# Whisper-6/DynamicTreeAttn

Hardware: AMD Instinct MI355X
Metric: tree-attn fwd+bwd tokens/sec, Qwen3-0.6B tau2-16k tries (higher is better)
Workload: dtype bf16

## Files before the change

### dynamictreeattn_amd/_lib.py

```python
from __future__ import annotations

import ctypes as C
import os

from .build import LIB

_lib = None
_i32, _i64, _f32, _vp = C.c_int32, C.c_int64, C.c_float, C.c_void_p

_PROTOS = {
    "dta_version": ([], C.c_int),
    "dta_take_pending_error": ([C.c_char_p, _i32], C.c_int),
    "dta_lcp_adjacent": ([_vp, _vp, _vp, _i32, _vp, _vp, _vp], C.c_int),
    "dta_leafize": ([_vp, _vp, _i32, _vp, _vp, _vp, _vp, _vp], C.c_int),
    "dta_preorder_meta": ([_vp] * 8 + [_i32, _i32] + [_vp] * 4 + [_vp], C.c_int),
    "dta_tree_attn_fwd": ([_vp] * 8 + [_i32] * 6 + [_i64] * 8 + [_f32, _i32] + [_vp, _i32, _f32, _vp], C.c_int),
    "dta_tree_attn_bwd": ([_vp] * 14 + [_i32] * 6 + [_i64] * 12 + [_f32, _i32, _i32, _i32] + [_vp, _i32, _vp, _i32, _vp]
                          + [_vp, _i32, _f32, _vp], C.c_int),
    "dta_window_lo": ([_vp] * 4 + [_i32, _i32, _i32, _vp, _vp], C.c_int),
    "dta_logprob_entropy_fwd": ([_vp] * 8 + [_i32, _i32, _i64, _f32, _i32, _f32, _vp], C.c_int),
    "dta_logprob_entropy_shard_stats": ([_vp] * 6 + [_i32, _i32, _i64, _f32, _i32, _f32, _vp], C.c_int),
    "dta_logprob_entropy_bwd": ([_vp] * 10 + [_i32, _i32, _i64, _i64, _f32, _i32, _f32, _vp], C.c_int),
    "dta_rmsnorm_fwd": ([_vp] * 6 + [_i32, _i32, _f32, _f32, _i32, _vp], C.c_int),
    "dta_rmsnorm_bwd_blocks": ([_i32], C.c_int),
    "dta_rmsnorm_bwd": ([_vp] * 7 + [_i32, _i32, _f32, _i32, _vp], C.c_int),
    "dta_qk_norm_rope_fwd": ([_vp] * 5 + [_i32, _i32, _i32, _i64, _f32, _i32, _vp], C.c_int),
    "dta_qk_norm_rope_bwd_blocks": ([_i64], C.c_int),
    "dta_qk_norm_rope_bwd": ([_vp] * 7 + [_i32, _i32, _i32, _i64, _i64, _i64, _i64, _i32, _vp], C.c_int),
    "dta_wide_qk_norm_rope_fwd": ([_vp] * 5 + [_i32, _i32, _i32, _i64, _f32, _i32, _vp], C.c_int),
    "dta_wide_qk_norm_rope_bwd_blocks": ([_i32], C.c_int),
    "dta_wide_qk_norm_rope_bwd": ([_vp] * 7 + [_i32, _i32, _i32, _i64, _i64, _i64, _i64, _i32, _vp], C.c_int),
    "dta_rmsnorm_add_fwd": ([_vp] * 6 + [_i32, _i32, _f32, _i32, _vp], C.c_int),
    "dta_swiglu_fwd": ([_vp] * 3 + [_i64, _i32, _i64, _i32, _vp], C.c_int),
    "dta_swiglu_bwd": ([_vp] * 5 + [_i64, _i32, _i64, _i64, _i32, _vp], C.c_int),
    "dta_geglu_fwd": ([_vp] * 3 + [_i64, _i32, _i64, _i32, _vp], C.c_int),
    "dta_geglu_bwd": ([_vp] * 5 + [_i64, _i32, _i64, _i64, _i32, _vp], C.c_int),
    "dta_transpose": ([_vp, _vp, _i64, _i64, _i64, _i64, _i32, _vp], C.c_int),
    "dta_sum_slabs": ([_vp, _i64, _i64, _i64, _vp, _vp, _i32, _vp], C.c_int),
    "dta_moe_router_fwd": ([_vp] * 4 + [_i32] * 5 + [_vp], C.c_int),
    "dta_moe_router_bwd": ([_vp] * 5 + [_i32] * 5 + [_vp], C.c_int),
    "dta_moe_permute_workspace": ([_i32, _i32], C.c_int),
    "dta_moe_tile_bound": ([_i32, _i32], C.c_int),
    "dta_moe_permute": ([_vp, _i32, _i32, _i32] + [_vp] * 5 + [_vp], C.c_int),
    "dta_moe_grouped_gemm": ([_i32] + [_vp] * 7 + [_i32] * 5 + [_vp], C.c_int),
    "dta_moe_combine_fwd": ([_vp] * 4 + [_i32] * 4 + [_vp], C.c_int),
    "dta_moe_combine_bwd": ([_vp] * 6 + [_i32] * 4 + [_vp], C.c_int),
    "dta_lora_down": ([_vp, _i64, _vp, _i64, _vp, _i64, _vp, _i32, _i32, _i32, _i32, _vp], C.c_int),
    "dta_lora_wgrad_slabs": ([_i32, _i32], C.c_int),
    "dta_lora_wgrad": ([_vp, _i64, _vp, _i64, _vp, _vp, _i32, _i32, _i32, _i32, _vp], C.c_int),
}
EXPORTS = tuple(_PROTOS)
_ERR = {-1: "DTA_EINVAL", -2: "DTA_EUNSUPPORTED", -3: "DTA_EALIGN", -4: "DTA_ELAUNCH", -5: "DTA_EPRIOR"}


def _hip_runtimes_mapped():
    try:
        with open("/proc/self/maps") as f:
            return sorted({line.split()[-1] for line in f if "libamdhip64" in line})
    except OSError:
        return []

# ... 34 lines not shown
```

### dynamictreeattn_amd/csrc/elementwise_kernels.hip

```cpp
#include <hip/hip_runtime.h>
#include <stdint.h>
#include "dta_common.h"
#include "dta_device.h"

#ifndef DTA_EW_NT
#define DTA_EW_NT 1
#endif
#if DTA_EW_NT
#define DTA_SAVED_LOAD(P) __builtin_nontemporal_load(P)
#else
#define DTA_SAVED_LOAD(P) (*(P))
#endif

namespace {


template <int DT, int NA, bool OFF = false>
__global__ __launch_bounds__(256) void rmsnorm_fwd_kernel(const void* __restrict__ x_, const void* __restrict__ delta_, const void* __restrict__ w_,
                                                          void* __restrict__ xout_, void* __restrict__ y_,
                                                          float* __restrict__ rstd, int R, int H, float eps, float w_off = 0.f) {
  using e = typename Ty<DT>::e; using v8 = typename Ty<DT>::v8;
  const int lane = threadIdx.x & 63, wave = threadIdx.x >> 6;
  const e* w = reinterpret_cast<const e*>(w_);
  const int nv = H >> 3;
// ... 135 lines not shown
    }
  }
  if (!dw_part) return;
  float* out = dw_part + (int64_t)blockIdx.x * H;
#pragma unroll
  for (int a = 0; a < NA; ++a) {
    if (a < per_lane) {
      __syncthreads();
#pragma unroll
      for (int j = 0; j < 8; ++j) red[(wave * 64 + lane) * 8 + j] = acc[a][j];
      __syncthreads();
      if (wave == 0) {
        const int i = lane + 64 * a;
        if (i < nv) {
#pragma unroll
          for (int j = 0; j < 8; ++j) out[8 * i + j] = red[lane * 8 + j] + red[(64 + lane) * 8 + j] + red[(128 + lane) * 8 + j] + red[(192 + lane) * 8 + j];
        }
      }
    }
  }
}

template <int DT, int HPL, int D>
__global__ __launch_bounds__(256) void qk_norm_rope_fwd_kernel(const void* __restrict__ x_, const void* __restrict__ w_, const float* __restrict__ cs,
                                                               void* __restrict__ y_, float* __restrict__ rstd, int64_t n_units, int NH,
                                                               int64_t x_st, float eps) {
  using e = typename Ty<DT>::e; using v8 = typename Ty<DT>::v8;
  constexpr int LPH = D / 8, LSH = D == 128 ? 4 : 3;
  const int lane = threadIdx.x & 63, sub = lane & (LPH - 1);
  const int64_t unit = ((int64_t)blockIdx.x * 4 + (threadIdx.x >> 6)) * (64 / LPH) + (lane >> LSH);
  if (unit >= n_units) return;
  const int groups = NH / HPL;
  const int64_t tok = unit / groups; const int head0 = (int)(unit - tok * groups) * HPL;
  const e* x = reinterpret_cast<const e*>(x_) + tok * x_st + (int64_t)head0 * D + 8 * sub;
  const int64_t hid0 = tok * NH + head0;
  e* y = reinterpret_cast<e*>(y_) + hid0 * D + 8 * sub;
  v8 v[HPL];
#pragma unroll
  for (int h = 0; h < HPL; ++h) v[h] = *reinterpret_cast<const v8*>(x + h * D);
  const float* c = cs + tok * D + 8 * (sub & (LPH / 2 - 1));
  float cj[8], sj[8];
#pragma unroll
  for (int j = 0; j < 8; ++j) { cj[j] = c[j]; sj[j] = sub < LPH / 2 ? -c[D / 2 + j] : c[D / 2 + j]; }
  v8 wv;
  if (w_) wv = *reinterpret_cast<const v8*>(reinterpret_cast<const e*>(w_) + 8 * sub);
#pragma unroll
  for (int h = 0; h < HPL; ++h) {
    float a[8];
    if (w_) {
      float ss = 0.f;
#pragma unroll
      for (int j = 0; j < 8; ++j) { const float f = (float)v[h][j]; ss = __builtin_fmaf(f, f, ss); }
#pragma unroll
      for (int o = LPH / 2; o > 0; o >>= 1) ss += __shfl_xor(ss, o);
      const float r = __builtin_amdgcn_rsqf(ss * (1.f / D) + eps);
      if (sub == 0) rstd[hid0 + h] = r;
#pragma unroll
      for (int j = 0; j < 8; ++j) { const e t = (e)((float)v[h][j] * r); a[j] = (float)(e)((float)wv[j] * (float)t); }
    } else {
#pragma unroll
      for (int j = 0; j < 8; ++j) a[j] = (float)v[h][j];
    }
    v8 o;
#pragma unroll
    for (int j = 0; j < 8; ++j) {
      const float other = __shfl_xor(a[j], LPH / 2);
      o[j] = (e)(a[j] * cj[j] + other * sj[j]);
    }
    *reinterpret_cast<v8*>(y + h * D) = o;
  }
}

template <int DT, int HPL, int D>
__global__ __launch_bounds__(256) void qk_norm_rope_bwd_kernel(const void* __restrict__ x_, const void* __restrict__ w_, const float* __restrict__ cs,
                                                               const void* dy_, const float* __restrict__ rstd,
                                                               void* dx_, float* __restrict__ dw_part, int64_t n_units, int NH,
                                                               int64_t x_st, int64_t dy_st_t, int64_t dy_st_h, int64_t dx_st) {
  using e = typename Ty<DT>::e; using v8 = typename Ty<DT>::v8;
  constexpr int LPH = D / 8, LSH = D == 128 ? 4 : 3, UPB = 4 * (64 / LPH);
  __shared__ float red[256 * 8];
  const int lane = threadIdx.x & 63, sub = lane & (LPH - 1);
  const int groups = NH / HPL;
  float acc[8];
#pragma unroll
  for (int j = 0; j < 8; ++j) acc[j] = 0.f;
  v8 wv;
  if (w_) wv = *reinterpret_cast<const v8*>(reinterpret_cast<const e*>(w_) + 8 * sub);
  for (int64_t base = (int64_t)blockIdx.x * UPB; base < n_units; base += (int64_t)gridDim.x * UPB) {
    const int64_t unit = base + (threadIdx.x >> 6) * (64 / LPH) + (lane >> LSH);
    const bool live = unit < n_units;
    const int64_t uc = live ? unit : n_units - 1;
    const int64_t tok = uc / groups; const int head0 = (int)(uc - tok * groups) * HPL;
    const e* dy = reinterpret_cast<const e*>(dy_) + tok * dy_st_t + (int64_t)head0 * dy_st_h + 8 * sub;
    v8 g[HPL], v[HPL];
#pragma unroll
    for (int h = 0; h < HPL; ++h) g[h] = *reinterpret_cast<const v8*>(dy + h * dy_st_h);
    if (w_) {
      const e* x = reinterpret_cast<const e*>(x_) + tok * x_st + (int64_t)head0 * D + 8 * sub;
#pragma unroll
      for (int h = 0; h < HPL; ++h) v[h] = DTA_SAVED_LOAD(reinterpret_cast<const v8*>(x + h * D));
    }
    const float* c = cs + tok * D + 8 * (sub & (LPH / 2 - 1));
    float cj[8], sj[8];
#pragma unroll
    for (int j = 0; j < 8; ++j) { cj[j] = c[j]; sj[j] = sub < LPH / 2 ? c[D / 2 + j] : -c[D / 2 + j]; }
    e* dx = reinterpret_cast<e*>(dx_) + tok * dx_st + (int64_t)head0 * D + 8 * sub;
#pragma unroll
    for (int h = 0; h < HPL; ++h) {
      float da[8];
#pragma unroll
      for (int j = 0; j < 8; ++j) {
// ... 7 lines not shown
        float dot = 0.f, t[8];
#pragma unroll
        for (int j = 0; j < 8; ++j) { t[j] = (float)v[h][j] * r; dot = __builtin_fmaf(da[j] * (float)wv[j], t[j], dot); if (live) acc[j] = __builtin_fmaf(da[j], t[j], acc[j]); }
#pragma unroll
        for (int o2 = LPH / 2; o2 > 0; o2 >>= 1) dot += __shfl_xor(dot, o2);
        dot *= (1.f / D);
#pragma unroll
        for (int j = 0; j < 8; ++j) o[j] = (e)(r * (da[j] * (float)wv[j] - t[j] * dot));
      } else {
#pragma unroll
        for (int j = 0; j < 8; ++j) o[j] = (e)da[j];
      }
      if (live) *reinterpret_cast<v8*>(dx + h * D) = o;
    }
  }
  if (w_ && dw_part) {
#pragma unroll
    for (int j = 0; j < 8; ++j) red[threadIdx.x * 8 + j] = acc[j];
    __syncthreads();
    if (threadIdx.x < D) {
      const int s = threadIdx.x >> 3, j = threadIdx.x & 7;
      float t = 0.f;
      for (int g2 = 0; g2 < 256 / LPH; ++g2) t += red[(g2 * LPH + s) * 8 + j];
      dw_part[(int64_t)blockIdx.x * D + threadIdx.x] = t;
    }
  }
}

template <int WPT> __device__ __forceinline__ float token_sum(float v, float* slot) {
  v = wave_sum(v);
  if constexpr (WPT == 1) return v;
  else {
    if ((threadIdx.x & 63) == 0) slot[threadIdx.x >> 6] = v;
    __syncthreads();
    const float t = (slot[0] + slot[1]) + (slot[2] + slot[3]);
    __syncthreads();
    return t;
  }
}

template <int DT, int NA, int D, int WPT>
__global__ __launch_bounds__(256) void wide_qk_norm_rope_fwd_kernel(const void* __restrict__ x_, const void* __restrict__ w_, const float* __restrict__ cs,
                                                                    void* __restrict__ y_, float* __restrict__ rstd, int T, int n,
                                                                    int64_t x_st, float eps) {
  using e = typename Ty<DT>::e; using v8 = typename Ty<DT>::v8;
  constexpr int LPH = D / 8, L = 64 * WPT, TPB = 4 / WPT;
  __shared__ float slot[4];
  const int lane = WPT == 1 ? (threadIdx.x & 63) : threadIdx.x, sub = lane & (LPH - 1);
  const e* w = reinterpret_cast<const e*>(w_);
// ... 355 lines not shown
  if (wave == 0 && col < n) {
    float t = extra ? extra[col] : 0.f;
#pragma unroll
    for (int w = 0; w < 16; ++w) t += red[w * 64 + lane];
    reinterpret_cast<e*>(out_)[col] = (e)t;
  }
}
template <int DT>
__global__ __launch_bounds__(256) void sum_slabs_flat_kernel(const float* __restrict__ part, int slabs, int64_t n4, int64_t stride,
                                                             const float* __restrict__ extra, void* __restrict__ out_) {
  using e = typename Ty<DT>::e;
  typedef float f4 __attribute__((ext_vector_type(4)));
  typedef e e4 __attribute__((ext_vector_type(4)));
  for (int64_t i = (int64_t)blockIdx.x * 256 + threadIdx.x; i < n4; i += (int64_t)gridDim.x * 256) {
    f4 t = extra ? *reinterpret_cast<const f4*>(extra + 4 * i) : f4{0.f, 0.f, 0.f, 0.f};
    for (int s2 = 0; s2 < slabs; ++s2) t += *reinterpret_cast<const f4*>(part + s2 * stride + 4 * i);
    e4 o;
#pragma unroll
    for (int j = 0; j < 4; ++j) o[j] = (e)t[j];
    *reinterpret_cast<e4*>(reinterpret_cast<e*>(out_) + 4 * i) = o;
  }
}

template <int N> using Int = std::integral_constant<int, N>;

template <int WIDE, class F> inline void rms_form(int H, float w_offset, F&& f) {
  auto by_h = [&](auto off) {
    if (H <= 1024) f(Int<2>{}, off);
    else if (H <= 2048) f(Int<4>{}, off);
    else if (H <= 4096) f(Int<8>{}, off);
    else f(Int<WIDE>{}, off);
  };
  if (w_offset != 0.f) by_h(std::true_type{}); else by_h(std::false_type{});
}

template <class F> inline void qk_form(int NH, int head_dim, F&& f) {
  if (head_dim == 64) { if (NH % 4 == 0) f(Int<4>{}, Int<64>{}); else f(Int<1>{}, Int<64>{}); }
  else if (NH % 4 == 0) f(Int<4>{}, Int<128>{}); else f(Int<1>{}, Int<128>{});
}

template <class F> inline void wide_qk_form(int64_t n, int head_dim, F&& f) {
  auto by_n = [&](auto d) {
    if (n <= 1024) f(Int<2>{}, d, Int<1>{});
    else if (n <= 2048) f(Int<4>{}, d, Int<1>{});
    else if (n <= 4096) f(Int<2>{}, d, Int<4>{});
    else f(Int<4>{}, d, Int<4>{});
// ... 81 lines not shown
      hipLaunchKernelGGL((qk_norm_rope_fwd_kernel<decltype(dt)::value, HPL, D>), grid, block, 0, st_, x, w, cos_sin, y, rstd, n, NH, x_stride_t, eps);
    });
  });
  return DTA_LAUNCH_STATUS();
}

extern "C" int dta_qk_norm_rope_bwd_blocks(int64_t n_heads_total) { return row_blocks(n_heads_total, 16, 1024); }
extern "C" int dta_qk_norm_rope_bwd(const void* x, const void* w, const float* cos_sin, const void* dy, const float* rstd,
                                    void* dx, float* dw_partial, int32_t T, int32_t NH, int32_t head_dim,
                                    int64_t x_stride_t, int64_t dy_stride_t, int64_t dy_stride_h, int64_t dx_stride_t, int32_t dtype, void* stream) {
  if (!cos_sin || !dy || !dx || T <= 0 || NH <= 0 || (w && (!x || !rstd))) return DTA_EINVAL;
  if (!row_dtype_ok(dtype) || (head_dim != 128 && head_dim != 64)) return DTA_EUNSUPPORTED;
  if (!aligned16(dy) || !aligned16(dx) || (w && (!aligned16(w) || !aligned16(x))) || x_stride_t % 8 || dy_stride_t % 8 || dy_stride_h % 8 || dx_stride_t % 8) return DTA_EALIGN;
  if (dx_stride_t < (int64_t)NH * head_dim) return DTA_EINVAL;
  hipStream_t st_ = static_cast<hipStream_t>(stream);
  DTA_REFUSE_IF_PRIOR_ERROR();
  const dim3 grid(row_blocks((int64_t)T * NH, 16, 1024)), block(256);
  qk_form(NH, head_dim, [&](auto hpl, auto d) {
    constexpr int HPL = decltype(hpl)::value, D = decltype(d)::value;
    const int64_t n = (int64_t)T * (NH / HPL);
    dta_storage_type(dtype, [&](auto dt) {
      hipLaunchKernelGGL((qk_norm_rope_bwd_kernel<decltype(dt)::value, HPL, D>), grid, block, 0, st_, x, w, cos_sin, dy, rstd, dx, dw_partial, n, NH,
                         x_stride_t, dy_stride_t, dy_stride_h, dx_stride_t);
    });
  });
  return DTA_LAUNCH_STATUS();
}

extern "C" int dta_wide_qk_norm_rope_fwd(const void* x, const void* w, const float* cos_sin, void* y, float* rstd,
                                         int32_t T, int32_t NH, int32_t head_dim, int64_t x_stride_t, float eps, int32_t dtype, void* stream) {
  if (!x || !w || !cos_sin || !y || !rstd || T <= 0 || NH <= 0 || eps != eps) return DTA_EINVAL;
  if (!row_dtype_ok(dtype) || (head_dim != 128 && head_dim != 64) || (int64_t)NH * head_dim > 8192) return DTA_EUNSUPPORTED;
  if (!aligned16(x) || !aligned16(w) || !aligned16(y) || x_stride_t % 8) return DTA_EALIGN;
  const int n = NH * head_dim;
  if (x_stride_t < n) return DTA_EINVAL;
  hipStream_t st_ = static_cast<hipStream_t>(stream);
  DTA_REFUSE_IF_PRIOR_ERROR();
  const dim3 grid(row_blocks(T, 4, 8192)), block(256);
  wide_qk_form(n, head_dim, [&](auto na, auto d, auto wpt) {
    dta_storage_type(dtype, [&](auto dt) {
      hipLaunchKernelGGL((wide_qk_norm_rope_fwd_kernel<decltype(dt)::value, decltype(na)::value, decltype(d)::value, decltype(wpt)::value>), grid, block, 0, st_,
                         x, w, cos_sin, y, rstd, T, n, x_stride_t, eps);
    });
  });
  return DTA_LAUNCH_STATUS();
}
// ... 67 lines not shown
}

extern "C" int dta_sum_slabs(const float* part, int64_t slabs, int64_t n, int64_t slab_stride, const float* extra, void* out, int32_t out_dtype,
                             void* stream) {
  if (!part || !out || slabs <= 0 || n <= 0 || slab_stride < n) return DTA_EINVAL;
  if (!row_dtype_ok(out_dtype)) return DTA_EUNSUPPORTED;
  hipStream_t st_ = static_cast<hipStream_t>(stream);
  DTA_REFUSE_IF_PRIOR_ERROR();
  const bool flat = slabs <= 16 && n % 4 == 0 && slab_stride % 4 == 0 && aligned16(part) && aligned16(out) && (!extra || aligned16(extra));
  if (flat) {
    const dim3 grid(row_blocks(n / 4, 256, 8192)), block(256);
    dta_storage_type(out_dtype, [&](auto dt) {
      hipLaunchKernelGGL(sum_slabs_flat_kernel<decltype(dt)::value>, grid, block, 0, st_, part, (int)slabs, n / 4, slab_stride, extra, out);
    });
  } else {
    if ((n + 63) / 64 > 0x7fffffff) return DTA_EUNSUPPORTED;
    const dim3 grid((unsigned)((n + 63) / 64)), block(1024);
    dta_storage_type(out_dtype, [&](auto dt) {
      hipLaunchKernelGGL(sum_slabs_tall_kernel<decltype(dt)::value>, grid, block, 0, st_, part, slabs, n, slab_stride, extra, out);
    });
  }
  return DTA_LAUNCH_STATUS();
}
```

### dynamictreeattn_amd/ops.py

```python
from __future__ import annotations

import math
from dataclasses import dataclass
from typing import Optional

import numpy as np
import torch
import torch.nn.functional as F

from . import packing
from ._lib import check, lib, ptr

_DT = {torch.bfloat16: 0, torch.float16: 1, torch.float32: 2}


class _on:
    __slots__ = ("dev", "_guard")

    def __init__(self, *ts):
        dev = None
        for t in ts:
            if t is None:
                continue
            if not t.is_cuda:
# ... 603 lines not shown
    return sum_slabs(part, w.dtype) if part is not None else None


def _qk_norm_rope_fwd(x, w, cos_sin, eps):
    T, NH, D = x.shape
    y = torch.empty((T, NH, D), dtype=x.dtype, device=x.device)
    rstd = torch.empty(T * NH, dtype=torch.float32, device=x.device) if w is not None else None
    _launch("dta_qk_norm_rope_fwd", (x, w, cos_sin), ptr(x), ptr(w), ptr(cos_sin), ptr(y), ptr(rstd), T, NH, D, x.stride(0), float(eps),
            _DT[x.dtype], nbytes=2 * T * NH * D * x.element_size() + T * D * 4)
    return y, rstd


def _qk_norm_rope_bwd(x, w, cos_sin, dy, rstd, dx, need_w):
    T, NH, D = x.shape
    if dy.stride(2) != 1:
        dy = dy.contiguous()
    part = torch.empty(lib().dta_qk_norm_rope_bwd_blocks(T * NH), D, dtype=torch.float32, device=x.device) if w is not None and need_w else None
    _launch("dta_qk_norm_rope_bwd", (x, cos_sin, dy), ptr(x), ptr(w), ptr(cos_sin), ptr(dy), ptr(rstd) if w is not None else None,
            ptr(dx), ptr(part), T, NH, D, x.stride(0), dy.stride(0), dy.stride(1), dx.stride(0), _DT[x.dtype],
            nbytes=(3 if w is not None else 2) * T * NH * D * x.element_size() + T * D * 4)
    return sum_slabs(part, w.dtype) if part is not None else None


class _QKNormRope(torch.autograd.Function):
    @staticmethod
    def forward(ctx, x, w, cos_sin, eps):
        _require_cuda(x, cos_sin)
        T, NH, D = x.shape
        if x.stride(2) != 1 or x.stride(1) != D:
            x = x.contiguous()
        y, rstd = _qk_norm_rope_fwd(x, w, cos_sin, eps)
        ctx.save_for_backward(x, w if w is not None else cos_sin, cos_sin, rstd if rstd is not None else cos_sin)
        ctx.has_w = w is not None
        return y

    @staticmethod
    def backward(ctx, dy):
        x, w, cos_sin, rstd = ctx.saved_tensors
        dx = torch.empty(x.shape, dtype=x.dtype, device=x.device)
        dw = _qk_norm_rope_bwd(x, w if ctx.has_w else None, cos_sin, dy, rstd, dx, ctx.needs_input_grad[1])
        return dx, dw, None, None


class _QKVPrep(torch.autograd.Function):

    @staticmethod
    def forward(ctx, qkv, wq, wk, cos_sin, eps, Hq, Hkv, wide=False):
        _require_cuda(qkv, cos_sin)
        T, H3, D = qkv.shape
        assert H3 == Hq + 2 * Hkv and qkv.is_contiguous()
        assert not wide or (wq is not None and wk is not None)
        ctx.wide = bool(wide)
        fwd = _wide_qk_norm_rope_fwd if wide else _qk_norm_rope_fwd
        outs, rstds = [], []
        for x, w in ((qkv[:, :Hq], wq), (qkv[:, Hq:Hq + Hkv], wk)):
            y, rstd = fwd(x, w, cos_sin, eps)
            outs.append(y); rstds.append(rstd if rstd is not None else cos_sin)
        ctx.save_for_backward(qkv, wq if wq is not None else cos_sin, wk if wk is not None else cos_sin, cos_sin, rstds[0], rstds[1])
        ctx.has_w = (wq is not None, wk is not None)
        ctx.heads = (Hq, Hkv)
        return outs[0], outs[1], qkv[:, Hq + Hkv:]

    @staticmethod
    def backward(ctx, dq, dk, dv):
        qkv, wq, wk, cos_sin, rq, rk = ctx.saved_tensors
        Hq, Hkv = ctx.heads
        T, H3, D = qkv.shape
        base = dv._base
        in_place = (base is not None and dq._base is base and dk._base is base and base.shape == qkv.shape and base.is_contiguous()
                    and base.dtype == qkv.dtype and dq.shape == (T, Hq, D) and dk.shape == (T, Hkv, D) and dv.shape == (T, Hkv, D)
                    and dq.stride() == dk.stride() == dv.stride() == (H3 * D, D, 1)
                    and (dq.storage_offset(), dk.storage_offset(), dv.storage_offset()) == (0, Hq * D, (Hq + Hkv) * D))
        d = base if in_place else torch.empty_like(qkv)
        dws = []
        for lo, NH, w, rstd, has_w, need_w, dy in ((0, Hq, wq, rq, ctx.has_w[0], ctx.needs_input_grad[1], dq),
                                                   (Hq, Hkv, wk, rk, ctx.has_w[1], ctx.needs_input_grad[2], dk)):
            bwd = _wide_qk_norm_rope_bwd if ctx.wide else _qk_norm_rope_bwd
            dws.append(bwd(qkv[:, lo:lo + NH], w if has_w else None, cos_sin, dy, rstd, d[:, lo:lo + NH], need_w))
        if not in_place:
            d[:, Hq + Hkv:].copy_(dv)
        return d, dws[0], dws[1], None, None, None, None, None


def qkv_prep(qkv: torch.Tensor, wq: Optional[torch.Tensor], wk: Optional[torch.Tensor], cos_sin: torch.Tensor, eps: float,
             Hq: int, Hkv: int):
    return _QKVPrep.apply(qkv, wq, wk, cos_sin, eps, Hq, Hkv)


def qkv_prep_wide(qkv: torch.Tensor, wq: torch.Tensor, wk: torch.Tensor, cos_sin: torch.Tensor, eps: float, Hq: int, Hkv: int):
    return _QKVPrep.apply(qkv, wq, wk, cos_sin, eps, Hq, Hkv, True)


def qk_norm_rope(x: torch.Tensor, w: Optional[torch.Tensor], cos_sin: torch.Tensor, eps: float) -> torch.Tensor:
    return _QKNormRope.apply(x, w, cos_sin, eps)


ROPE_TYPES = ("default", "linear", "llama3", "yarn")


def rope_inv_freq(D: int, rope_parameters: dict, max_position_embeddings: Optional[int] = None):
    rp = rope_parameters
# ... 168 lines not shown
        outs, o = [], 0
        for r in ctx.rows:
            outs.append(g[o:o + r]); o += r
        return tuple(outs)


def stack_rows(*ws: torch.Tensor) -> torch.Tensor:
    return _StackRows.apply(*ws)


def clear_stack_rows_cache() -> None:
    _StackRows._cache.clear(); _StackRows._cached_bytes = 0


def sum_slabs(part: torch.Tensor, out_dtype: torch.dtype, extra: torch.Tensor = None) -> torch.Tensor:
    assert part.dtype == torch.float32 and part.is_contiguous() and (extra is None or (extra.dtype == torch.float32 and extra.is_contiguous()))
    S, n = part.shape[0], part[0].numel()
    assert extra is None or extra.numel() == n
    out = torch.empty(part.shape[1:], dtype=out_dtype, device=part.device)
    _launch("dta_sum_slabs", (part, extra, out), ptr(part), S, n, n, ptr(extra), ptr(out), _DT[out_dtype], nbytes=(S + (extra is not None)) * n * 4)
    return out


def transpose_2d(w: torch.Tensor) -> torch.Tensor:
    R, C = w.shape
    if w.stride(1) != 1:
        w = w.contiguous()
    out = torch.empty((C, R), dtype=w.dtype, device=w.device)
    _launch("dta_transpose", (w, out), ptr(w), ptr(out), R, C, w.stride(0), R, w.element_size(), nbytes=2 * R * C * w.element_size())
    return out


class _TransposedWeights:
    cache: dict = {}
    nbytes = 0

    @staticmethod
    def get(w: torch.Tensor) -> torch.Tensor:
        if weight_cache.depth == 0:
            return transpose_2d(w)
        key = (w.data_ptr(), tuple(w.shape), w.dtype, w._version)
        hit = _TransposedWeights.cache.get(key)
        if hit is not None:
            return hit
        wt = transpose_2d(w)
        n = wt.numel() * wt.element_size()
# ... 8 lines not shown


def _dgrad(dy: torch.Tensor, w: torch.Tensor) -> torch.Tensor:
    if dy.is_cuda and w.dtype in (torch.bfloat16, torch.float16) and dy.shape[0] >= 4096 and w.shape[0] % 8 == 0 and w.shape[1] % 8 == 0:
        return dy @ _TransposedWeights.get(w).t()
    return dy @ w


WGRAD_SPLIT_K = 4


def _wgrad(x: torch.Tensor, dy: torch.Tensor, transposed: bool) -> torch.Tensor:
    T = x.shape[0]
    a, b = (x, dy) if transposed else (dy, x)
    S = WGRAD_SPLIT_K
    tiles = -(-a.shape[1] // 256) * -(-b.shape[1] // 256)
    per = (T // S) // 64 * 64
    if tiles > 64 or per < 2048 or not x.is_cuda or x.dtype == torch.float32:
        out = a.t() @ b
    else:
        body = per * S
        part = torch.bmm(a[:body].reshape(S, per, a.shape[1]).transpose(1, 2), b[:body].reshape(S, per, b.shape[1]), out_dtype=torch.float32)
        rest = torch.mm(a[body:].t(), b[body:], out_dtype=torch.float32) if body < T else None
        out = sum_slabs(part, x.dtype, rest)
    if not transposed:
        return out
    V = 16 // out.element_size()
    return transpose_2d(out) if out.is_cuda and out.shape[0] % V == 0 and out.shape[1] % V == 0 else out.t()


class _Linear(torch.autograd.Function):

    @staticmethod
    def forward(ctx, x, w, b):
        ctx.save_for_backward(x, w)
        ctx.has_bias = b is not None
        return F.linear(x, w, b)

    @staticmethod
    def backward(ctx, dy):
        x, w = ctx.saved_tensors
        dx = _dgrad(dy, w) if ctx.needs_input_grad[0] else None
        dw = None
        if ctx.needs_input_grad[1]:
            dw = _wgrad(x, dy, w.shape[1] >= 2 * w.shape[0])
        db = dy.sum(0) if ctx.has_bias and ctx.needs_input_grad[2] else None
# ... 289 lines not shown
```

### include/dta.h

```cpp
#ifndef DTA_H
#define DTA_H
#include <stdint.h>

#ifdef __cplusplus
extern "C" {
#endif

#define DTA_OK 0
#define DTA_EINVAL (-1)
#define DTA_EUNSUPPORTED (-2)
#define DTA_EALIGN (-3)
#define DTA_ELAUNCH (-4)
#define DTA_EPRIOR (-5)

#define DTA_BF16 0
#define DTA_F16 1
#define DTA_F32 2

#define DTA_QTILE 128
#define DTA_KTILE 128

int dta_version(void);

int dta_take_pending_error(char* msg, int32_t cap);
// ... 42 lines not shown
                            float* lse, float* entropy, float* logprob, float* extra_logprob,
                            int32_t R, int32_t V, int64_t row_stride, float temperature, int32_t dtype, float softcap, void* stream);
int dta_logprob_entropy_shard_stats(const void* logits, const int64_t* labels, const int32_t* extra_ptr, const int64_t* extra_labels,
                                    float* stats, float* extra_picked,
                                    int32_t R, int32_t V, int64_t row_stride, float temperature, int32_t dtype, float softcap, void* stream);
int dta_logprob_entropy_bwd(const void* logits, void* dlogits, const int64_t* labels, const int32_t* extra_ptr, const int64_t* extra_labels,
                            const float* lse, const float* entropy,
                            const float* g_logprob, const float* g_extra_logprob, const float* g_entropy,
                            int32_t R, int32_t V, int64_t row_stride, int64_t out_row_stride, float temperature, int32_t dtype,
                            float softcap, void* stream);

int dta_rmsnorm_fwd(const void* x, const void* delta, const void* w, void* x_out, void* y, float* rstd,
                    int32_t R, int32_t H, float eps, float w_offset, int32_t dtype, void* stream);
int dta_rmsnorm_bwd_blocks(int32_t R);
int dta_rmsnorm_bwd(const void* x, const void* w, const void* dy, const void* dres, const float* rstd, void* dx, float* dw_partial,
                    int32_t R, int32_t H, float w_offset, int32_t dtype, void* stream);
int dta_qk_norm_rope_fwd(const void* x, const void* w, const float* cos_sin, void* y, float* rstd,
                         int32_t T, int32_t NH, int32_t head_dim, int64_t x_stride_t, float eps, int32_t dtype, void* stream);
int dta_qk_norm_rope_bwd_blocks(int64_t n_heads_total);
int dta_qk_norm_rope_bwd(const void* x, const void* w, const float* cos_sin, const void* dy, const float* rstd,
                         void* dx, float* dw_partial, int32_t T, int32_t NH, int32_t head_dim,
                         int64_t x_stride_t, int64_t dy_stride_t, int64_t dy_stride_h, int64_t dx_stride_t,
                         int32_t dtype, void* stream);
int dta_wide_qk_norm_rope_fwd(const void* x, const void* w, const float* cos_sin, void* y, float* rstd,
                              int32_t T, int32_t NH, int32_t head_dim, int64_t x_stride_t, float eps, int32_t dtype, void* stream);
int dta_wide_qk_norm_rope_bwd_blocks(int32_t T);
int dta_wide_qk_norm_rope_bwd(const void* x, const void* w, const float* cos_sin, const void* dy, const float* rstd,
                              void* dx, float* dw_partial, int32_t T, int32_t NH, int32_t head_dim,
                              int64_t x_stride_t, int64_t dy_stride_t, int64_t dy_stride_h, int64_t dx_stride_t,
                              int32_t dtype, void* stream);
int dta_rmsnorm_add_fwd(const void* y, const void* w, const void* res, void* out, void* yn, float* rstd,
                        int32_t R, int32_t H, float eps, int32_t dtype, void* stream);
int dta_swiglu_fwd(const void* gate, const void* up, void* y, int64_t rows, int32_t cols, int64_t ld, int32_t dtype, void* stream);
int dta_swiglu_bwd(const void* gate, const void* up, const void* dy, void* dgate, void* dup,
                   int64_t rows, int32_t cols, int64_t ld, int64_t ld_grad, int32_t dtype, void* stream);
int dta_geglu_fwd(const void* gate, const void* up, void* y, int64_t rows, int32_t cols, int64_t ld, int32_t dtype, void* stream);
int dta_geglu_bwd(const void* gate, const void* up, const void* dy, void* dgate, void* dup,
                  int64_t rows, int32_t cols, int64_t ld, int64_t ld_grad, int32_t dtype, void* stream);

int dta_transpose(const void* in, void* out, int64_t rows, int64_t cols, int64_t ld_in, int64_t ld_out, int32_t elem_size, void* stream);

int dta_sum_slabs(const float* part, int64_t slabs, int64_t n, int64_t slab_stride, const float* extra, void* out, int32_t out_dtype, void* stream);

#define DTA_MOE_BM 128
#define DTA_MOE_FWD 0
#define DTA_MOE_DGRAD 1
#define DTA_MOE_WGRAD 2

int dta_moe_router_fwd(const void* logits, int32_t* topk_ids, void* topk_w, float* lse, int32_t T, int32_t E, int32_t k, int32_t norm_topk,
                       int32_t dtype, void* stream);
int dta_moe_router_bwd(const void* logits, const float* lse, const int32_t* topk_ids, const void* dtopk_w, void* dlogits,
                       int32_t T, int32_t E, int32_t k, int32_t norm_topk, int32_t dtype, void* stream);

int dta_moe_permute_workspace(int32_t n_pairs, int32_t E);
int dta_moe_tile_bound(int32_t n_pairs, int32_t E);
int dta_moe_permute(const int32_t* topk_ids, int32_t T, int32_t k, int32_t E, int32_t* workspace,
                    int32_t* expert_offsets, int32_t* row_of_pair, int32_t* src_token, int32_t* tiles, void* stream);

int dta_moe_grouped_gemm(int32_t mode, const void* x, const void* w, const void* dy, void* out, const int32_t* gather,
                         const int32_t* expert_offsets, const int32_t* tiles, int32_t n_rows, int32_t E, int32_t N, int32_t K,
                         int32_t dtype, void* stream);

int dta_moe_combine_fwd(const void* y, const void* topk_w, const int32_t* row_of_pair, void* out, int32_t T, int32_t k, int32_t H,
                        int32_t dtype, void* stream);
int dta_moe_combine_bwd(const void* dout, const void* y, const void* topk_w, const int32_t* row_of_pair, void* dy, void* dtopk_w,
// ... 13 lines not shown
```

Measured before the change: 883,700.

## Fuse Q/K norm-rope launches and fold transpose into slab-sum epilogue

Adds single-launch Q+K norm-rope forward and backward kernels that split the grid between Q and K heads, replacing two separate launches per direction. It also adds a sum_slabs_t kernel that reduces fp32 weight-gradient slabs and writes the transposed result through a shared-memory tile, removing a separate transpose pass in the LoRA/linear wgrad path. Both are enabled by a FUSED_EPILOGUES flag. The cost is added code paths and a fallback to the two-launch path when the head counts differ in divisibility by 4.

```diff
diff --git a/dynamictreeattn_amd/_lib.py b/dynamictreeattn_amd/_lib.py
--- a/dynamictreeattn_amd/_lib.py
+++ b/dynamictreeattn_amd/_lib.py
@@ -27,6 +27,8 @@
     "dta_qk_norm_rope_fwd": ([_vp] * 5 + [_i32, _i32, _i32, _i64, _f32, _i32, _vp], C.c_int),
     "dta_qk_norm_rope_bwd_blocks": ([_i64], C.c_int),
     "dta_qk_norm_rope_bwd": ([_vp] * 7 + [_i32, _i32, _i32, _i64, _i64, _i64, _i64, _i32, _vp], C.c_int),
+    "dta_qk_norm_rope2_fwd": ([_vp] * 8 + [_i32, _i32, _i32, _i32, _i64, _f32, _i32, _vp], C.c_int),
+    "dta_qk_norm_rope2_bwd": ([_vp] * 11 + [_i32, _i32, _i32, _i32] + [_i64] * 6 + [_i32, _vp], C.c_int),
     "dta_wide_qk_norm_rope_fwd": ([_vp] * 5 + [_i32, _i32, _i32, _i64, _f32, _i32, _vp], C.c_int),
     "dta_wide_qk_norm_rope_bwd_blocks": ([_i32], C.c_int),
     "dta_wide_qk_norm_rope_bwd": ([_vp] * 7 + [_i32, _i32, _i32, _i64, _i64, _i64, _i64, _i32, _vp], C.c_int),
@@ -37,6 +39,7 @@
     "dta_geglu_bwd": ([_vp] * 5 + [_i64, _i32, _i64, _i64, _i32, _vp], C.c_int),
     "dta_transpose": ([_vp, _vp, _i64, _i64, _i64, _i64, _i32, _vp], C.c_int),
     "dta_sum_slabs": ([_vp, _i64, _i64, _i64, _vp, _vp, _i32, _vp], C.c_int),
+    "dta_sum_slabs_t": ([_vp, _i64, _i64, _i64, _i64, _vp, _vp, _i32, _vp], C.c_int),
     "dta_moe_router_fwd": ([_vp] * 4 + [_i32] * 5 + [_vp], C.c_int),
     "dta_moe_router_bwd": ([_vp] * 5 + [_i32] * 5 + [_vp], C.c_int),
     "dta_moe_permute_workspace": ([_i32, _i32], C.c_int),
diff --git a/dynamictreeattn_amd/csrc/elementwise_kernels.hip b/dynamictreeattn_amd/csrc/elementwise_kernels.hip
--- a/dynamictreeattn_amd/csrc/elementwise_kernels.hip
+++ b/dynamictreeattn_amd/csrc/elementwise_kernels.hip
@@ -181,13 +181,13 @@
 }
 
 template <int DT, int HPL, int D>
-__global__ __launch_bounds__(256) void qk_norm_rope_fwd_kernel(const void* __restrict__ x_, const void* __restrict__ w_, const float* __restrict__ cs,
-                                                               void* __restrict__ y_, float* __restrict__ rstd, int64_t n_units, int NH,
-                                                               int64_t x_st, float eps) {
+__device__ __forceinline__ void qk_norm_rope_fwd_body(const void* __restrict__ x_, const void* __restrict__ w_, const float* __restrict__ cs,
+                                                      void* __restrict__ y_, float* __restrict__ rstd, int64_t n_units, int NH,
+                                                      int64_t x_st, float eps, unsigned bid) {
   using e = typename Ty<DT>::e; using v8 = typename Ty<DT>::v8;
   constexpr int LPH = D / 8, LSH = D == 128 ? 4 : 3;
   const int lane = threadIdx.x & 63, sub = lane & (LPH - 1);
-  const int64_t unit = ((int64_t)blockIdx.x * 4 + (threadIdx.x >> 6)) * (64 / LPH) + (lane >> LSH);
+  const int64_t unit = ((int64_t)bid * 4 + (threadIdx.x >> 6)) * (64 / LPH) + (lane >> LSH);
   if (unit >= n_units) return;
   const int groups = NH / HPL;
   const int64_t tok = unit / groups; const int head0 = (int)(unit - tok * groups) * HPL;
@@ -231,13 +231,20 @@
 }
 
 template <int DT, int HPL, int D>
-__global__ __launch_bounds__(256) void qk_norm_rope_bwd_kernel(const void* __restrict__ x_, const void* __restrict__ w_, const float* __restrict__ cs,
-                                                               const void* dy_, const float* __restrict__ rstd,
-                                                               void* dx_, float* __restrict__ dw_part, int64_t n_units, int NH,
-                                                               int64_t x_st, int64_t dy_st_t, int64_t dy_st_h, int64_t dx_st) {
+__global__ __launch_bounds__(256) void qk_norm_rope_fwd_kernel(const void* __restrict__ x_, const void* __restrict__ w_, const float* __restrict__ cs,
+                                                               void* __restrict__ y_, float* __restrict__ rstd, int64_t n_units, int NH,
+                                                               int64_t x_st, float eps) {
+  qk_norm_rope_fwd_body<DT, HPL, D>(x_, w_, cs, y_, rstd, n_units, NH, x_st, eps, blockIdx.x);
+}
+
+template <int DT, int HPL, int D>
+__device__ __forceinline__ void qk_norm_rope_bwd_body(const void* __restrict__ x_, const void* __restrict__ w_, const float* __restrict__ cs,
+                                                      const void* dy_, const float* __restrict__ rstd,
+                                                      void* dx_, float* __restrict__ dw_part, int64_t n_units, int NH,
+                                                      int64_t x_st, int64_t dy_st_t, int64_t dy_st_h, int64_t dx_st, unsigned bid, unsigned nblk,
+                                                      float* red) {
   using e = typename Ty<DT>::e; using v8 = typename Ty<DT>::v8;
   constexpr int LPH = D / 8, LSH = D == 128 ? 4 : 3, UPB = 4 * (64 / LPH);
-  __shared__ float red[256 * 8];
   const int lane = threadIdx.x & 63, sub = lane & (LPH - 1);
   const int groups = NH / HPL;
   float acc[8];
@@ -245,7 +252,7 @@
   for (int j = 0; j < 8; ++j) acc[j] = 0.f;
   v8 wv;
   if (w_) wv = *reinterpret_cast<const v8*>(reinterpret_cast<const e*>(w_) + 8 * sub);
-  for (int64_t base = (int64_t)blockIdx.x * UPB; base < n_units; base += (int64_t)gridDim.x * UPB) {
+  for (int64_t base = (int64_t)bid * UPB; base < n_units; base += (int64_t)nblk * UPB) {
     const int64_t unit = base + (threadIdx.x >> 6) * (64 / LPH) + (lane >> LSH);
     const bool live = unit < n_units;
     const int64_t uc = live ? unit : n_units - 1;
@@ -299,9 +306,41 @@
       const int s = threadIdx.x >> 3, j = threadIdx.x & 7;
       float t = 0.f;
       for (int g2 = 0; g2 < 256 / LPH; ++g2) t += red[(g2 * LPH + s) * 8 + j];
-      dw_part[(int64_t)blockIdx.x * D + threadIdx.x] = t;
-    }
-  }
+      dw_part[(int64_t)bid * D + threadIdx.x] = t;
+    }
+  }
+}
+
+template <int DT, int HPL, int D>
+__global__ __launch_bounds__(256) void qk_norm_rope_bwd_kernel(const void* __restrict__ x_, const void* __restrict__ w_, const float* __restrict__ cs,
+                                                               const void* dy_, const float* __restrict__ rstd,
+                                                               void* dx_, float* __restrict__ dw_part, int64_t n_units, int NH,
+                                                               int64_t x_st, int64_t dy_st_t, int64_t dy_st_h, int64_t dx_st) {
+  __shared__ float red[256 * 8];
+  qk_norm_rope_bwd_body<DT, HPL, D>(x_, w_, cs, dy_, rstd, dx_, dw_part, n_units, NH, x_st, dy_st_t, dy_st_h, dx_st, blockIdx.x, gridDim.x, red);
+}
+
+struct QkSide {
+  const void* x; const void* w; const void* dy; void* out; float* rstd; float* dw_part;
+  int64_t n_units, dy_st_t, dy_st_h;
+  int NH; unsigned nblk;
+};
+
+template <int DT, int HPL, int D>
+__global__ __launch_bounds__(256) void qk_norm_rope2_fwd_kernel(QkSide q, QkSide k, const float* __restrict__ cs, int64_t x_st, float eps) {
+  const bool is_q = blockIdx.x < q.nblk;
+  qk_norm_rope_fwd_body<DT, HPL, D>(is_q ? q.x : k.x, is_q ? q.w : k.w, cs, is_q ? q.out : k.out, is_q ? q.rstd : k.rstd,
+                                    is_q ? q.n_units : k.n_units, is_q ? q.NH : k.NH, x_st, eps, is_q ? blockIdx.x : blockIdx.x - q.nblk);
+}
+
+template <int DT, int HPL, int D>
+__global__ __launch_bounds__(256) void qk_norm_rope2_bwd_kernel(QkSide q, QkSide k, const float* __restrict__ cs, int64_t x_st, int64_t dx_st) {
+  __shared__ float red[256 * 8];
+  const bool is_q = blockIdx.x < q.nblk;
+  qk_norm_rope_bwd_body<DT, HPL, D>(is_q ? q.x : k.x, is_q ? q.w : k.w, cs, is_q ? q.dy : k.dy, is_q ? q.rstd : k.rstd, is_q ? q.out : k.out,
+                                    is_q ? q.dw_part : k.dw_part, is_q ? q.n_units : k.n_units, is_q ? q.NH : k.NH, x_st,
+                                    is_q ? q.dy_st_t : k.dy_st_t, is_q ? q.dy_st_h : k.dy_st_h, dx_st, is_q ? blockIdx.x : blockIdx.x - q.nblk,
+                                    is_q ? q.nblk : k.nblk, red);
 }
 
 template <int WPT> __device__ __forceinline__ float token_sum(float v, float* slot) {
@@ -703,6 +742,68 @@
   }
 }
 
+template <int DT>
+__global__ __launch_bounds__(256) void sum_slabs_t_kernel(const float* __restrict__ part, int slabs, int64_t rows, int64_t cols, int64_t stride,
+                                                          const float* __restrict__ extra, char* __restrict__ out) {
+  using e = typename Ty<DT>::e;
+  typedef float f4 __attribute__((ext_vector_type(4)));
+  constexpr int ESZ = sizeof(e), TS = 64;
+  constexpr int WPR = ESZ == 2 ? TS / 2 : TS;
+  constexpr int PITCH = WPR + 4;
+  __shared__ __attribute__((aligned(16))) uint32_t tile[TS * PITCH];
+  const int64_t r0 = (int64_t)blockIdx.y * TS, c0 = (int64_t)blockIdx.x * TS;
+  const int tid = threadIdx.x;
+  auto sum4 = [&](int64_t i) -> f4 {
+    f4 t = extra ? *reinterpret_cast<const f4*>(extra + i) : f4{0.f, 0.f, 0.f, 0.f};
+    for (int s2 = 0; s2 < slabs; ++s2) t += *reinterpret_cast<const f4*>(part + s2 * stride + i);
+    return t;
+  };
+  if constexpr (ESZ == 2) {
+    auto bits = [](float f) -> uint32_t { return (uint32_t)__builtin_bit_cast(uint16_t, (e)f); };
+    const int rp = tid >> 3, ch = tid & 7, r = 2 * rp, c = 8 * ch;
+    uint32_t aw[4] = {0, 0, 0, 0}, bw[4] = {0, 0, 0, 0};
+    if (c0 + c < cols) {
+      if (r0 + r < rows) {
+        const int64_t i = (r0 + r) * cols + c0 + c;
+        const f4 lo = sum4(i), hi = sum4(i + 4);
+        aw[0] = bits(lo[0]) | (bits(lo[1]) << 16); aw[1] = bits(lo[2]) | (bits(lo[3]) << 16);
+        aw[2] = bits(hi[0]) | (bits(hi[1]) << 16); aw[3] = bits(hi[2]) | (bits(hi[3]) << 16);
+      }
+      if (r0 + r + 1 < rows) {
+        const int64_t i = (r0 + r + 1) * cols + c0 + c;
+        const f4 lo = sum4(i), hi = sum4(i + 4);
+        bw[0] = bits(lo[0]) | (bits(lo[1]) << 16); bw[1] = bits(lo[2]) | (bits(lo[3]) << 16);
+        bw[2] = bits(hi[0]) | (bits(hi[1]) << 16); bw[3] = bits(hi[2]) | (bits(hi[3]) << 16);
+      }
+    }
+#pragma unroll
+    for (int j = 0; j < 4; ++j) {
+      tile[(c + 2 * j) * PITCH + rp] = (aw[j] & 0xffffu) | (bw[j] << 16);
+      tile[(c + 2 * j + 1) * PITCH + rp] = (aw[j] >> 16) | (bw[j] & 0xffff0000u);
+    }
+    __syncthreads();
+    for (int i = tid; i < TS * 8; i += 256) {
+      const int oc = i >> 3, k = i & 7;
+      if (c0 + oc < cols && r0 + 8 * k < rows)
+        *reinterpret_cast<uint4*>(out + ((c0 + oc) * rows + r0 + 8 * k) * 2) = *reinterpret_cast<const uint4*>(&tile[oc * PITCH + 4 * k]);
+    }
+  } else {
+    for (int i = tid; i < TS * 16; i += 256) {
+      const int r = i >> 4, c = 4 * (i & 15);
+      f4 a = {0.f, 0.f, 0.f, 0.f};
+      if (r0 + r < rows && c0 + c < cols) a = sum4((r0 + r) * cols + c0 + c);
+#pragma unroll
+      for (int j = 0; j < 4; ++j) { const float aj = a[j]; tile[(c + j) * PITCH + r] = __float_as_uint(aj); }
+    }
+    __syncthreads();
+    for (int i = tid; i < TS * 16; i += 256) {
+      const int oc = i >> 4, k = i & 15;
+      if (c0 + oc < cols && r0 + 4 * k < rows)
+        *reinterpret_cast<uint4*>(out + ((c0 + oc) * rows + r0 + 4 * k) * 4) = *reinterpret_cast<const uint4*>(&tile[oc * PITCH + 4 * k]);
+    }
+  }
+}
+
 template <int N> using Int = std::integral_constant<int, N>;
 
 template <int WIDE, class F> inline void rms_form(int H, float w_offset, F&& f) {
@@ -830,6 +931,70 @@
     dta_storage_type(dtype, [&](auto dt) {
       hipLaunchKernelGGL((qk_norm_rope_bwd_kernel<decltype(dt)::value, HPL, D>), grid, block, 0, st_, x, w, cos_sin, dy, rstd, dx, dw_partial, n, NH,
                          x_stride_t, dy_stride_t, dy_stride_h, dx_stride_t);
+    });
+  });
+  return DTA_LAUNCH_STATUS();
+}
+
+extern "C" int dta_qk_norm_rope2_fwd(const void* qkv, const void* wq, const void* wk, const float* cos_sin, void* y_q, void* y_k,
+                                     float* rstd_q, float* rstd_k, int32_t T, int32_t Hq, int32_t Hkv, int32_t head_dim, int64_t x_stride_t,
+                                     float eps, int32_t dtype, void* stream) {
+  if (!qkv || !cos_sin || !y_q || !y_k || T <= 0 || Hq <= 0 || Hkv <= 0 || (wq && !rstd_q) || (wk && !rstd_k)) return DTA_EINVAL;
+  if (!row_dtype_ok(dtype) || (head_dim != 128 && head_dim != 64)) return DTA_EUNSUPPORTED;
+  if (!aligned16(qkv) || !aligned16(y_q) || !aligned16(y_k) || (wq && !aligned16(wq)) || (wk && !aligned16(wk)) || x_stride_t % 8) return DTA_EALIGN;
+  if (x_stride_t < (int64_t)(Hq + Hkv) * head_dim) return DTA_EINVAL;
+  const void* xk = (const char*)qkv + (int64_t)Hq * head_dim * (dtype == DTA_F32 ? 4 : 2);
+  if ((Hq % 4 == 0) != (Hkv % 4 == 0)) {
+    const int st = dta_qk_norm_rope_fwd(qkv, wq, cos_sin, y_q, rstd_q, T, Hq, head_dim, x_stride_t, eps, dtype, stream);
+    return st != DTA_OK ? st : dta_qk_norm_rope_fwd(xk, wk, cos_sin, y_k, rstd_k, T, Hkv, head_dim, x_stride_t, eps, dtype, stream);
+  }
+  hipStream_t st_ = static_cast<hipStream_t>(stream);
+  DTA_REFUSE_IF_PRIOR_ERROR();
+  qk_form(Hq, head_dim, [&](auto hpl, auto d) {
+    constexpr int HPL = decltype(hpl)::value, D = decltype(d)::value, UPB = 4 * (64 / (D / 8));
+    QkSide q{}, k{};
+    q.x = qkv; q.w = wq; q.out = y_q; q.rstd = rstd_q; q.NH = Hq; q.n_units = (int64_t)T * (Hq / HPL);
+    k.x = xk; k.w = wk; k.out = y_k; k.rstd = rstd_k; k.NH = Hkv; k.n_units = (int64_t)T * (Hkv / HPL);
+    q.nblk = (unsigned)((q.n_units + UPB - 1) / UPB); k.nblk = (unsigned)((k.n_units + UPB - 1) / UPB);
+    dta_storage_type(dtype, [&](auto dt) {
+      hipLaunchKernelGGL((qk_norm_rope2_fwd_kernel<decltype(dt)::value, HPL, D>), dim3(q.nblk + k.nblk), dim3(256), 0, st_, q, k, cos_sin, x_stride_t, eps);
+    });
+  });
+  return DTA_LAUNCH_STATUS();
+}
+
+extern "C" int dta_qk_norm_rope2_bwd(const void* qkv, const void* wq, const void* wk, const float* cos_sin, const void* dy_q, const void* dy_k,
+                                     const float* rstd_q, const float* rstd_k, void* dx, float* dwq_partial, float* dwk_partial,
+                                     int32_t T, int32_t Hq, int32_t Hkv, int32_t head_dim, int64_t x_stride_t,
+                                     int64_t dyq_stride_t, int64_t dyq_stride_h, int64_t dyk_stride_t, int64_t dyk_stride_h, int64_t dx_stride_t,
+                                     int32_t dtype, void* stream) {
+  if (!cos_sin || !dy_q || !dy_k || !dx || T <= 0 || Hq <= 0 || Hkv <= 0 || ((wq || wk) && !qkv) || (wq && !rstd_q) || (wk && !rstd_k)) return DTA_EINVAL;
+  if (!row_dtype_ok(dtype) || (head_dim != 128 && head_dim != 64)) return DTA_EUNSUPPORTED;
+  if (!aligned16(dy_q) || !aligned16(dy_k) || !aligned16(dx) || (wq && !aligned16(wq)) || (wk && !aligned16(wk)) || (qkv && !aligned16(qkv)) ||
+      x_stride_t % 8 || dyq_stride_t % 8 || dyq_stride_h % 8 || dyk_stride_t % 8 || dyk_stride_h % 8 || dx_stride_t % 8) return DTA_EALIGN;
+  if (dx_stride_t < (int64_t)(Hq + Hkv) * head_dim || (qkv && x_stride_t < (int64_t)(Hq + Hkv) * head_dim)) return DTA_EINVAL;
+  const int64_t koff = (int64_t)Hq * head_dim * (dtype == DTA_F32 ? 4 : 2);
+  const void* xk = qkv ? (const char*)qkv + koff : nullptr;
+  void* dxk = (char*)dx + koff;
+  if ((Hq % 4 == 0) != (Hkv % 4 == 0)) {
+    const int st = dta_qk_norm_rope_bwd(qkv, wq, cos_sin, dy_q, rstd_q, dx, dwq_partial, T, Hq, head_dim, x_stride_t, dyq_stride_t, dyq_stride_h,
+                                        dx_stride_t, dtype, stream);
+    return st != DTA_OK ? st : dta_qk_norm_rope_bwd(xk, wk, cos_sin, dy_k, rstd_k, dxk, dwk_partial, T, Hkv, head_dim, x_stride_t, dyk_stride_t,
+                                                    dyk_stride_h, dx_stride_t, dtype, stream);
+  }
+  hipStream_t st_ = static_cast<hipStream_t>(stream);
+  DTA_REFUSE_IF_PRIOR_ERROR();
+  qk_form(Hq, head_dim, [&](auto hpl, auto d) {
+    constexpr int HPL = decltype(hpl)::value, D = decltype(d)::value;
+    QkSide q{}, k{};
+    q.x = qkv; q.w = wq; q.dy = dy_q; q.out = dx; q.rstd = const_cast<float*>(rstd_q); q.dw_part = dwq_partial; q.NH = Hq;
+    q.n_units = (int64_t)T * (Hq / HPL); q.dy_st_t = dyq_stride_t; q.dy_st_h = dyq_stride_h;
+    k.x = xk; k.w = wk; k.dy = dy_k; k.out = dxk; k.rstd = const_cast<float*>(rstd_k); k.dw_part = dwk_partial; k.NH = Hkv;
+    k.n_units = (int64_t)T * (Hkv / HPL); k.dy_st_t = dyk_stride_t; k.dy_st_h = dyk_stride_h;
+    q.nblk = (unsigned)row_blocks((int64_t)T * Hq, 16, 1024); k.nblk = (unsigned)row_blocks((int64_t)T * Hkv, 16, 1024);
+    dta_storage_type(dtype, [&](auto dt) {
+      hipLaunchKernelGGL((qk_norm_rope2_bwd_kernel<decltype(dt)::value, HPL, D>), dim3(q.nblk + k.nblk), dim3(256), 0, st_, q, k, cos_sin, x_stride_t,
+                         dx_stride_t);
     });
   });
   return DTA_LAUNCH_STATUS();
@@ -943,3 +1108,20 @@
   }
   return DTA_LAUNCH_STATUS();
 }
+
+extern "C" int dta_sum_slabs_t(const float* part, int64_t slabs, int64_t rows, int64_t cols, int64_t slab_stride, const float* extra, void* out,
+                               int32_t out_dtype, void* stream) {
+  if (!part || !out || slabs <= 0 || rows <= 0 || cols <= 0 || rows > (int64_t)1 << 40 || cols > (int64_t)1 << 20 || slab_stride < rows * cols) return DTA_EINVAL;
+  if (!row_dtype_ok(out_dtype) || slabs > 16) return DTA_EUNSUPPORTED;
+  const int V = out_dtype == DTA_F32 ? 4 : 8;
+  if (rows % V || cols % V || slab_stride % 4) return DTA_EUNSUPPORTED;
+  if (!aligned16(part) || !aligned16(out) || (extra && !aligned16(extra))) return DTA_EALIGN;
+  hipStream_t st_ = static_cast<hipStream_t>(stream);
+  DTA_REFUSE_IF_PRIOR_ERROR();
+  const dim3 grid((unsigned)((cols + 63) / 64), (unsigned)((rows + 63) / 64)), block(256);
+  if (grid.y > 65535) return DTA_EUNSUPPORTED;
+  dta_storage_type(out_dtype, [&](auto dt) {
+    hipLaunchKernelGGL(sum_slabs_t_kernel<decltype(dt)::value>, grid, block, 0, st_, part, (int)slabs, rows, cols, slab_stride, extra, (char*)out);
+  });
+  return DTA_LAUNCH_STATUS();
+}
diff --git a/dynamictreeattn_amd/ops.py b/dynamictreeattn_amd/ops.py
--- a/dynamictreeattn_amd/ops.py
+++ b/dynamictreeattn_amd/ops.py
@@ -649,6 +649,31 @@
     return sum_slabs(part, w.dtype) if part is not None else None
 
 
+FUSED_EPILOGUES = True
+
+
+def _qk_norm_rope2_fwd(qkv, wq, wk, cos_sin, eps, Hq, Hkv):
+    T, _, D = qkv.shape
+    ys = [torch.empty((T, NH, D), dtype=qkv.dtype, device=qkv.device) for NH in (Hq, Hkv)]
+    rstds = [torch.empty(T * NH, dtype=torch.float32, device=qkv.device) if w is not None else None for NH, w in ((Hq, wq), (Hkv, wk))]
+    _launch("dta_qk_norm_rope2_fwd", (qkv, wq, wk, cos_sin), ptr(qkv), ptr(wq), ptr(wk), ptr(cos_sin), ptr(ys[0]), ptr(ys[1]), ptr(rstds[0]),
+            ptr(rstds[1]), T, Hq, Hkv, D, qkv.stride(0), float(eps), _DT[qkv.dtype],
+            nbytes=2 * T * (Hq + Hkv) * D * qkv.element_size() + T * D * 4)
+    return ys[0], ys[1], rstds[0], rstds[1]
+
+
+def _qk_norm_rope2_bwd(qkv, wq, wk, cos_sin, dq, dk, rq, rk, d, Hq, Hkv, need_wq, need_wk):
+    T, _, D = qkv.shape
+    dq, dk = (g if g.stride(2) == 1 else g.contiguous() for g in (dq, dk))
+    parts = [torch.empty(lib().dta_qk_norm_rope_bwd_blocks(T * NH), D, dtype=torch.float32, device=qkv.device) if w is not None and need else None
+             for NH, w, need in ((Hq, wq, need_wq), (Hkv, wk, need_wk))]
+    _launch("dta_qk_norm_rope2_bwd", (qkv, cos_sin, dq, dk, d), ptr(qkv), ptr(wq), ptr(wk), ptr(cos_sin), ptr(dq), ptr(dk),
+            ptr(rq) if wq is not None else None, ptr(rk) if wk is not None else None, ptr(d), ptr(parts[0]), ptr(parts[1]), T, Hq, Hkv, D,
+            qkv.stride(0), dq.stride(0), dq.stride(1), dk.stride(0), dk.stride(1), d.stride(0), _DT[qkv.dtype],
+            nbytes=(2 * (Hq + Hkv) + (Hq if wq is not None else 0) + (Hkv if wk is not None else 0)) * T * D * qkv.element_size() + T * D * 4)
+    return tuple(sum_slabs(part, w.dtype) if part is not None else None for part, w in ((parts[0], wq), (parts[1], wk)))
+
+
 class _QKNormRope(torch.autograd.Function):
     @staticmethod
     def forward(ctx, x, w, cos_sin, eps):
@@ -678,11 +703,15 @@
         assert H3 == Hq + 2 * Hkv and qkv.is_contiguous()
         assert not wide or (wq is not None and wk is not None)
         ctx.wide = bool(wide)
-        fwd = _wide_qk_norm_rope_fwd if wide else _qk_norm_rope_fwd
-        outs, rstds = [], []
-        for x, w in ((qkv[:, :Hq], wq), (qkv[:, Hq:Hq + Hkv], wk)):
-            y, rstd = fwd(x, w, cos_sin, eps)
-            outs.append(y); rstds.append(rstd if rstd is not None else cos_sin)
+        if FUSED_EPILOGUES and not wide:
+            yq, yk, rq, rk = _qk_norm_rope2_fwd(qkv, wq, wk, cos_sin, eps, Hq, Hkv)
+            outs, rstds = [yq, yk], [r if r is not None else cos_sin for r in (rq, rk)]
+        else:
+            fwd = _wide_qk_norm_rope_fwd if wide else _qk_norm_rope_fwd
+            outs, rstds = [], []
+            for x, w in ((qkv[:, :Hq], wq), (qkv[:, Hq:Hq + Hkv], wk)):
+                y, rstd = fwd(x, w, cos_sin, eps)
+                outs.append(y); rstds.append(rstd if rstd is not None else cos_sin)
         ctx.save_for_backward(qkv, wq if wq is not None else cos_sin, wk if wk is not None else cos_sin, cos_sin, rstds[0], rstds[1])
         ctx.has_w = (wq is not None, wk is not None)
         ctx.heads = (Hq, Hkv)
@@ -699,11 +728,15 @@
                     and dq.stride() == dk.stride() == dv.stride() == (H3 * D, D, 1)
                     and (dq.storage_offset(), dk.storage_offset(), dv.storage_offset()) == (0, Hq * D, (Hq + Hkv) * D))
         d = base if in_place else torch.empty_like(qkv)
-        dws = []
-        for lo, NH, w, rstd, has_w, need_w, dy in ((0, Hq, wq, rq, ctx.has_w[0], ctx.needs_input_grad[1], dq),
-                                                   (Hq, Hkv, wk, rk, ctx.has_w[1], ctx.needs_input_grad[2], dk)):
-            bwd = _wide_qk_norm_rope_bwd if ctx.wide else _qk_norm_rope_bwd
-            dws.append(bwd(qkv[:, lo:lo + NH], w if has_w else None, cos_sin, dy, rstd, d[:, lo:lo + NH], need_w))
+        if FUSED_EPILOGUES and not ctx.wide:
+            dws = _qk_norm_rope2_bwd(qkv, wq if ctx.has_w[0] else None, wk if ctx.has_w[1] else None, cos_sin, dq, dk, rq, rk, d, Hq, Hkv,
+                                     ctx.needs_input_grad[1], ctx.needs_input_grad[2])
+        else:
+            dws = []
+            for lo, NH, w, rstd, has_w, need_w, dy in ((0, Hq, wq, rq, ctx.has_w[0], ctx.needs_input_grad[1], dq),
+                                                       (Hq, Hkv, wk, rk, ctx.has_w[1], ctx.needs_input_grad[2], dk)):
+                bwd = _wide_qk_norm_rope_bwd if ctx.wide else _qk_norm_rope_bwd
+                dws.append(bwd(qkv[:, lo:lo + NH], w if has_w else None, cos_sin, dy, rstd, d[:, lo:lo + NH], need_w))
         if not in_place:
             d[:, Hq + Hkv:].copy_(dv)
         return d, dws[0], dws[1], None, None, None, None, None
@@ -918,6 +951,21 @@
     return out
 
 
+def sum_slabs_t_ok(S: int, R: int, C: int, out_dtype: torch.dtype) -> bool:
+    V = 128 // torch.finfo(out_dtype).bits
+    return S <= 16 and R % V == 0 and C % V == 0
+
+
+def sum_slabs_t(part: torch.Tensor, out_dtype: torch.dtype, extra: torch.Tensor = None) -> torch.Tensor:
+    assert part.dim() == 3 and part.dtype == torch.float32 and part.is_contiguous()
+    assert extra is None or (extra.dtype == torch.float32 and extra.is_contiguous() and extra.shape == part.shape[1:])
+    S, R, C = part.shape
+    out = torch.empty((C, R), dtype=out_dtype, device=part.device)
+    _launch("dta_sum_slabs_t", (part, extra, out), ptr(part), S, R, C, R * C, ptr(extra), ptr(out), _DT[out_dtype],
+            nbytes=(S + (extra is not None)) * R * C * 4 + R * C * out.element_size())
+    return out
+
+
 def transpose_2d(w: torch.Tensor) -> torch.Tensor:
     R, C = w.shape
     if w.stride(1) != 1:
@@ -972,6 +1020,8 @@
         body = per * S
         part = torch.bmm(a[:body].reshape(S, per, a.shape[1]).transpose(1, 2), b[:body].reshape(S, per, b.shape[1]), out_dtype=torch.float32)
         rest = torch.mm(a[body:].t(), b[body:], out_dtype=torch.float32) if body < T else None
+        if transposed and FUSED_EPILOGUES and sum_slabs_t_ok(S, part.shape[1], part.shape[2], x.dtype):
+            return sum_slabs_t(part, x.dtype, rest)
         out = sum_slabs(part, x.dtype, rest)
     if not transposed:
         return out
diff --git a/include/dta.h b/include/dta.h
--- a/include/dta.h
+++ b/include/dta.h
@@ -88,6 +88,14 @@
                          void* dx, float* dw_partial, int32_t T, int32_t NH, int32_t head_dim,
                          int64_t x_stride_t, int64_t dy_stride_t, int64_t dy_stride_h, int64_t dx_stride_t,
                          int32_t dtype, void* stream);
+int dta_qk_norm_rope2_fwd(const void* qkv, const void* wq, const void* wk, const float* cos_sin, void* y_q, void* y_k,
+                          float* rstd_q, float* rstd_k, int32_t T, int32_t Hq, int32_t Hkv, int32_t head_dim, int64_t x_stride_t,
+                          float eps, int32_t dtype, void* stream);
+int dta_qk_norm_rope2_bwd(const void* qkv, const void* wq, const void* wk, const float* cos_sin, const void* dy_q, const void* dy_k,
+                          const float* rstd_q, const float* rstd_k, void* dx, float* dwq_partial, float* dwk_partial,
+                          int32_t T, int32_t Hq, int32_t Hkv, int32_t head_dim, int64_t x_stride_t,
+                          int64_t dyq_stride_t, int64_t dyq_stride_h, int64_t dyk_stride_t, int64_t dyk_stride_h, int64_t dx_stride_t,
+                          int32_t dtype, void* stream);
 int dta_wide_qk_norm_rope_fwd(const void* x, const void* w, const float* cos_sin, void* y, float* rstd,
                               int32_t T, int32_t NH, int32_t head_dim, int64_t x_stride_t, float eps, int32_t dtype, void* stream);
 int dta_wide_qk_norm_rope_bwd_blocks(int32_t T);
@@ -107,6 +115,8 @@
 int dta_transpose(const void* in, void* out, int64_t rows, int64_t cols, int64_t ld_in, int64_t ld_out, int32_t elem_size, void* stream);
 
 int dta_sum_slabs(const float* part, int64_t slabs, int64_t n, int64_t slab_stride, const float* extra, void* out, int32_t out_dtype, void* stream);
+int dta_sum_slabs_t(const float* part, int64_t slabs, int64_t rows, int64_t cols, int64_t slab_stride, const float* extra, void* out,
+                    int32_t out_dtype, void* stream);
 
 #define DTA_MOE_BM 128
 #define DTA_MOE_FWD 0
```

Result: no change. 882,300 (median of 2 runs) (-0.2%).
